# hamaadshah/gan_deeplearning4j

Hardware: NVIDIA H100
Metric: images/sec (full G+D step) (higher is better)
Workload: dtype bf16

## Files before the change

gan_deeplearning4j_b200/csrc/kernels_ew.cu:

```cuda
#include <stdlib.h>
#include <algorithm>
#include "kernels.h"
#include "common.cuh"

namespace b2g {

uint64_t g_launch_count = 0;
const char* g_ew_last_kernel = "";

template <typename T>
__global__ void nchw_f32_to_nhwc_kernel(const float* __restrict__ src, T* __restrict__ dst, int N, int C, int HW) { pdl_enter();
  size_t total = (size_t)N * C * HW;
  for (size_t i = blockIdx.x * (size_t)blockDim.x + threadIdx.x; i < total; i += (size_t)gridDim.x * blockDim.x) {
    int c = i % C; size_t t = i / C; int p = t % HW; size_t n = t / HW;
    stf(dst, i, src[(n * C + c) * HW + p]);
  }
}
template <typename T>
__global__ void nhwc_to_nchw_f32_kernel(const T* __restrict__ src, float* __restrict__ dst, int N, int C, int HW) { pdl_enter();
  size_t total = (size_t)N * C * HW;
  for (size_t i = blockIdx.x * (size_t)blockDim.x + threadIdx.x; i < total; i += (size_t)gridDim.x * blockDim.x) {
    int p = i % HW; size_t t = i / HW; int c = t % C; size_t n = t / C;
    dst[i] = ldf(src, (n * HW + p) * C + c);
  }
}
template <typename T>
__global__ void permute_kernel(const T* __restrict__ src, T* __restrict__ dst, int N, int C, int HW, int to_nhwc) { pdl_enter();
  size_t total = (size_t)N * C * HW;
  for (size_t i = blockIdx.x * (size_t)blockDim.x + threadIdx.x; i < total; i += (size_t)gridDim.x * blockDim.x) {
    if (to_nhwc) { int c = i % C; size_t t = i / C; int p = t % HW; size_t n = t / HW; dst[i] = src[(n * C + c) * HW + p]; }
    else         { int p = i % HW; size_t t = i / HW; int c = t % C; size_t n = t / C; dst[i] = src[(n * HW + p) * C + c]; }
  }
}
#define DISPATCH_ACT(act, ACTC, ...)                                                            \
  switch (act) {                                                                                \
    case ACT_IDENTITY: { constexpr int ACTC = ACT_IDENTITY; __VA_ARGS__; } break;               \
    case ACT_RELU: { constexpr int ACTC = ACT_RELU; __VA_ARGS__; } break;                       \
    case ACT_LRELU: { constexpr int ACTC = ACT_LRELU; __VA_ARGS__; } break;                     \
    default: { constexpr int ACTC = -1; __VA_ARGS__; } break;                                   \
  }
int device_sm_count() {
  static int sms[64] = {}; int d = 0; cudaGetDevice(&d); if (d < 0 || d >= 64) d = 0;
  if (!sms[d]) { int v = 0; cudaDeviceGetAttribute(&v, cudaDevAttrMultiProcessorCount, d); sms[d] = v > 0 ? v : 1; }
  return sms[d];
}
static inline int vec4_blocks(size_t n_vec) { const size_t cap = (size_t)device_sm_count() * 4; size_t b = (n_vec + 1023) / 1024; if (b > cap) b = cap; if (b < 1) b = 1; return (int)b; }
static inline int ew_blocks(size_t n, int per = 256) { const size_t cap = (size_t)device_sm_count() * 16; size_t b = (n + per - 1) / per; if (b > cap) b = cap; if (b < 1) b = 1; return (int)b; }

void k_nchw_f32_to_nhwc(int prec, const float* src, void* dst, int N, int C, int HW, cudaStream_t s) {
  size_t n = (size_t)N * C * HW; if (!n) return;
  DISPATCH_PREC(prec, T, (launch_pdl(nchw_f32_to_nhwc_kernel<T>, dim3(ew_blocks(n)), dim3(256), (size_t)(0), s, src, (T*)dst, N, C, HW))); LAUNCHED();
}
void k_nhwc_to_nchw_f32(int prec, const void* src, float* dst, int N, int C, int HW, cudaStream_t s) {
  size_t n = (size_t)N * C * HW; if (!n) return;
  DISPATCH_PREC(prec, T, (launch_pdl(nhwc_to_nchw_f32_kernel<T>, dim3(ew_blocks(n)), dim3(256), (size_t)(0), s, (const T*)src, dst, N, C, HW))); LAUNCHED();
}
void k_permute(int prec, const void* src, void* dst, int N, int C, int HW, int to_nhwc, cudaStream_t s) {
  size_t n = (size_t)N * C * HW; if (!n) return;
  DISPATCH_PREC(prec, T, (launch_pdl(permute_kernel<T>, dim3(ew_blocks(n)), dim3(256), (size_t)(0), s, (const T*)src, (T*)dst, N, C, HW, to_nhwc))); LAUNCHED();
}
__global__ void cast_f32_to_bf16_kernel(const float* __restrict__ src, __nv_bfloat16* __restrict__ dst, size_t n) { pdl_enter();
  for (size_t i = blockIdx.x * (size_t)blockDim.x + threadIdx.x; i < n; i += (size_t)gridDim.x * blockDim.x) dst[i] = __float2bfloat16_rn(src[i]);
}
void k_cast_f32_to_bf16(const float* src, __nv_bfloat16* dst, size_t n, cudaStream_t s) {
  if (!n) return; launch_pdl(cast_f32_to_bf16_kernel, dim3(ew_blocks(n)), dim3(256), (size_t)(0), s, src, dst, n); LAUNCHED();
}
static const int SLICE_ELEMS = 1 << 20;
static inline int pick_slices(int rows, int C) {
  int cap = SLICE_ELEMS / (C > 0 ? C : 1); if (cap < 1) cap = 1; if (cap > 2048) cap = 2048;
  int S = rows / 8; if (S < 1) S = 1; if (S > cap) S = cap; return S;
}
size_t k_bn_scratch_floats(int C, int groups) { return (size_t)2 * groups * (SLICE_ELEMS + 2 * (size_t)C) + 64; }
size_t k_colsum_scratch_floats(int C) { return (size_t)(SLICE_ELEMS + C) + 64; }

__device__ __forceinline__ void unpack8(const uint4& u, float (&v)[8]) {
  const __nv_bfloat162* h = reinterpret_cast<const __nv_bfloat162*>(&u);
#pragma unroll
  for (int j = 0; j < 4; ++j) { float2 f = __bfloat1622float2(h[j]); v[2 * j] = f.x; v[2 * j + 1] = f.y; }
}
__device__ __forceinline__ uint4 pack8(const float (&v)[8]) {
  uint4 u; __nv_bfloat162* h = reinterpret_cast<__nv_bfloat162*>(&u);
#pragma unroll
  for (int j = 0; j < 4; ++j) h[j] = __floats2bfloat162_rn(v[2 * j], v[2 * j + 1]);
  return u;
}

template <typename T>
__global__ void bn_stats_partial_kernel(const T* __restrict__ x, int rows, int C, int S, float* __restrict__ psum, float* __restrict__ psq, float* __restrict__ pivot) { pdl_enter();
  int g = blockIdx.y;
  int idx = blockIdx.x * blockDim.x + threadIdx.x;
  if (idx >= S * C) return;
  int c = idx % C, sl = idx / C;
  const T* xg = x + (size_t)g * rows * C;
  const float k = ldf(xg, c);
  if (sl == 0) pivot[g * C + c] = k;
  float a = 0.f, b = 0.f;
  for (int r = sl; r < rows; r += S) { float v = ldf(xg, (size_t)r * C + c) - k; a += v; b = fmaf(v, v, b); }
  psum[((size_t)g * S + sl) * C + c] = a; psq[((size_t)g * S + sl) * C + c] = b;
}
static inline int vec_ty(int C) { int c8 = C / 8; int ty = 256 / c8; return ty < 1 ? 1 : ty; }
static inline bool vec_ok(int prec, int C) { return prec == PREC_BF16 && C % 8 == 0 && C / 8 <= 256 && 256 % (C / 8) == 0; }
static inline int vec_blocks(int rows, int C) { int ty = vec_ty(C); int b = rows / (ty * 4); int cap = SLICE_ELEMS / C; if (cap > 256) cap = 256; if (b > cap) b = cap; if (b < 1) b = 1; return b; }
template <int NV>
__device__ __forceinline__ void block_fold_write(float (&acc)[NV][8], int C, int C8, int c8, int ty, int TY, float* const (&dst)[NV], size_t row_off) {
  __shared__ float sred[NV][2048];
#pragma unroll
  for (int v = 0; v < NV; ++v)
#pragma unroll
    for (int j = 0; j < 8; ++j) sred[v][ty * C + c8 * 8 + j] = acc[v][j];
  __syncthreads();
  for (int c = threadIdx.x; c < C; c += blockDim.x) {
#pragma unroll
    for (int v = 0; v < NV; ++v) { float a = 0.f; for (int k = 0; k < TY; ++k) a += sred[v][k * C + c]; dst[v][row_off + c] = a; }
  }
}
__global__ void __launch_bounds__(1024) bn_stats_final_kernel(const float* __restrict__ psum, const float* __restrict__ psq, const float* __restrict__ pivot, int rows, int C, int S, int groups, float eps,
                                      float* __restrict__ mean, float* __restrict__ invstd,
                                      const float* __restrict__ run_mean, const float* __restrict__ run_var, float* g_mean, float* g_var, float decay) { pdl_enter();
  __shared__ double sa[32][33], sb[32][33];
  const int tx = threadIdx.x & 31, ty = threadIdx.x >> 5, c = blockIdx.x * 32 + tx;
  double acc_gm = 0.0, acc_gv = 0.0;
  for (int g = 0; g < groups; ++g) {
    double a = 0.0, b = 0.0;
    if (c < C) for (int sl0 = ty; sl0 < S; sl0 += 32 * 8) {
      float va[8], vb[8];
#pragma unroll
      for (int q = 0; q < 8; ++q) { const int sl = sl0 + 32 * q; va[q] = sl < S ? psum[((size_t)g * S + sl) * C + c] : 0.f; vb[q] = sl < S ? psq[((size_t)g * S + sl) * C + c] : 0.f; }
#pragma unroll
      for (int q = 0; q < 8; ++q) { a += va[q]; b += vb[q]; }
    }
    sa[ty][tx] = a; sb[ty][tx] = b;
    __syncthreads();
    if (ty == 0 && c < C) {
      for (int k = 1; k < 32; ++k) { a += sa[k][tx]; b += sb[k][tx]; }
      const double d = a / rows, mu = (double)pivot[g * C + c] + d; double var = b / rows - d * d; if (var < 0) var = 0;
      mean[g * C + c] = (float)mu; invstd[g * C + c] = (float)(1.0 / sqrt(var + (double)eps));
      if (g_mean) { acc_gm += (1.0 - decay) * ((double)run_mean[c] - mu); acc_gv += (1.0 - decay) * ((double)run_var[c] - var); }
    }
    __syncthreads();
  }
  if (g_mean && ty == 0 && c < C) { g_mean[c] = (float)(acc_gm / groups); g_var[c] = (float)(acc_gv / groups); }
}
void k_bn_stats(int prec, const void* x, int rows, int C, int groups, float* scratch, float* mean, float* invstd, float eps,
                const float* run_mean, const float* run_var, float* g_mean, float* g_var, float decay, cudaStream_t s) {
  const int S = pick_slices(rows, C);
  float* psum = scratch; float* psq = scratch + (size_t)groups * S * C; float* pivot = psq + (size_t)groups * S * C;
  dim3 grid((S * C + 255) / 256, groups);
  DISPATCH_PREC(prec, T, (launch_pdl(bn_stats_partial_kernel<T>, dim3(grid), dim3(256), (size_t)(0), s, (const T*)x, rows, C, S, psum, psq, pivot)));
  LAUNCHED();
  launch_pdl(bn_stats_final_kernel, dim3((C + 31) / 32), dim3(1024), (size_t)(0), s, psum, psq, (const float*)pivot, rows, C, S, groups, eps, mean, invstd, run_mean, run_var, g_mean, g_var, decay); LAUNCHED();
}
__global__ void bn_prep_infer_kernel(const float* __restrict__ rm, const float* __restrict__ rv, int C, int groups, float eps, float* mean, float* invstd) { pdl_enter();
  int i = blockIdx.x * blockDim.x + threadIdx.x; if (i >= C * groups) return;
  int c = i % C; mean[i] = rm[c]; invstd[i] = 1.0f / sqrtf(rv[c] + eps);
}
__global__ void bn_fold_kernel(const float* __restrict__ rm, const float* __restrict__ rv, const float* __restrict__ gamma, const float* __restrict__ beta, const float* __restrict__ cb, int C, float eps, float* scale, float* shift) { pdl_enter();
  int c = blockIdx.x * blockDim.x + threadIdx.x; if (c >= C) return;
  const float sc = gamma[c] / sqrtf(rv[c] + eps); scale[c] = sc; shift[c] = beta[c] - rm[c] * sc + (cb ? cb[c] * sc : 0.f);
}
void k_bn_fold(const float* rm, const float* rv, const float* gamma, const float* beta, const float* cb, int C, float eps, float* scale, float* shift, cudaStream_t s) {
  launch_pdl(bn_fold_kernel, dim3((C + 255) / 256), dim3(256), (size_t)0, s, rm, rv, gamma, beta, cb, C, eps, scale, shift); LAUNCHED();
}
void k_bn_prep_infer(const float* run_mean, const float* run_var, int C, int groups, float eps, float* mean, float* invstd, cudaStream_t s) {
  launch_pdl(bn_prep_infer_kernel, dim3((C * groups + 255) / 256), dim3(256), (size_t)(0), s, run_mean, run_var, C, groups, eps, mean, invstd); LAUNCHED();
}

template <typename T>
__global__ void bn_apply_kernel(const T* __restrict__ x, T* __restrict__ y, int rows, int C, int groups, const float* __restrict__ mean,
                                const float* __restrict__ invstd, const float* __restrict__ gamma, const float* __restrict__ beta, int act, float alpha) { pdl_enter();
  size_t per_group = (size_t)rows * C, total = per_group * groups;
  for (size_t i = blockIdx.x * (size_t)blockDim.x + threadIdx.x; i < total; i += (size_t)gridDim.x * blockDim.x) {
    int c = i % C; int g = i / per_group;
    float v = (ldf(x, i) - mean[g * C + c]) * invstd[g * C + c];
    stf(y, i, act_fwd(act, fmaf(gamma[c], v, beta[c]), alpha));
  }
}
template <int ACTC>
__global__ void __launch_bounds__(256, 3) bn_apply_bf16x8_kernel(const uint4* __restrict__ x, uint4* __restrict__ y, int rows, int C, int groups, const float* __restrict__ mean,
                                       const float* __restrict__ invstd, const float* __restrict__ gamma, const float* __restrict__ beta, int act, float alpha) { pdl_enter();
  const int C8 = C / 8; const size_t per_group = (size_t)rows * C8;
  const size_t t0 = blockIdx.x * (size_t)blockDim.x + threadIdx.x, stride = (size_t)gridDim.x * blockDim.x;
  const int c0 = (int)(t0 % C8) * 8;
  for (int g = 0; g < groups; ++g) {
    float mu[8], is[8], ga[8], be[8];
#pragma unroll
    for (int j = 0; j < 8; ++j) { mu[j] = mean[g * C + c0 + j]; is[j] = invstd[g * C + c0 + j]; ga[j] = gamma[c0 + j]; be[j] = beta[c0 + j]; }
    const uint4* xg = x + g * per_group; uint4* yg = y + g * per_group;
    for (size_t i = t0; i < per_group; i += 4 * stride) {
      uint4 xa[4];
#pragma unroll
      for (int q = 0; q < 4; ++q) if (i + q * stride < per_group) xa[q] = xg[i + q * stride];
#pragma unroll
      for (int q = 0; q < 4; ++q) if (i + q * stride < per_group) {
        float v[8]; unpack8(xa[q], v);
#pragma unroll
        for (int j = 0; j < 8; ++j) v[j] = act_fwd(ACTC < 0 ? act : ACTC, fmaf(ga[j], (v[j] - mu[j]) * is[j], be[j]), alpha);
        yg[i + q * stride] = pack8(v);
      }
    }
  }
}
void k_bn_apply(int prec, const void* x, void* y, int rows, int C, int groups, const float* mean, const float* invstd,
                const float* gamma, const float* beta, int act, float alpha, cudaStream_t s) {
  size_t n = (size_t)rows * C * groups; if (!n) return;
  if (vec_ok(prec, C)) {
    DISPATCH_ACT(act, ACTC, launch_pdl(bn_apply_bf16x8_kernel<ACTC>, dim3(vec4_blocks((size_t)rows * C / 8)), dim3(256), (size_t)(0), s, (const uint4*)x, (uint4*)y, rows, C, groups, mean, invstd, gamma, beta, act, alpha));
  } else {
    DISPATCH_PREC(prec, T, (launch_pdl(bn_apply_kernel<T>, dim3(ew_blocks(n)), dim3(256), (size_t)(0), s, (const T*)x, (T*)y, rows, C, groups, mean, invstd, gamma, beta, act, alpha)));
  }
  LAUNCHED();
}

template <typename T>
__global__ void bn_bwd_partial_kernel(const T* __restrict__ x, const T* __restrict__ eo, int rows, int C, int S, const float* __restrict__ mean,
                                      const float* __restrict__ invstd, const float* __restrict__ gamma, const float* __restrict__ beta, int act, float alpha,
                                      float* __restrict__ p1, float* __restrict__ p2) { pdl_enter();
  int g = blockIdx.y;
  int idx = blockIdx.x * blockDim.x + threadIdx.x;
  if (idx >= S * C) return;
  int c = idx % C, sl = idx / C;
  const T* xg = x + (size_t)g * rows * C; const T* eg = eo + (size_t)g * rows * C;
  float mu = mean[g * C + c], is = invstd[g * C + c], ga = gamma[c], be = beta[c];
  float a = 0.f, b = 0.f;
  for (int r = sl; r < rows; r += S) {
    float xh = (ldf(xg, (size_t)r * C + c) - mu) * is;
    float dy = ldf(eg, (size_t)r * C + c) * act_grad_from_pre(act, fmaf(ga, xh, be), alpha);
    a += dy; b = fmaf(dy, xh, b);
  }
  p1[((size_t)g * S + sl) * C + c] = a; p2[((size_t)g * S + sl) * C + c] = b;
}
__global__ void __launch_bounds__(1024) bn_bwd_final_kernel(const float* __restrict__ p1, const float* __restrict__ p2, int rows, int C, int S, int groups,
                                    float* __restrict__ c1, float* __restrict__ c2, float* g_gamma, float* g_beta, int want) { pdl_enter();
  __shared__ double sa[32][33], sb[32][33];
  const int tx = threadIdx.x & 31, ty = threadIdx.x >> 5, c = blockIdx.x * 32 + tx;
  double tg = 0.0, tb = 0.0;
  for (int g = 0; g < groups; ++g) {
    double a = 0.0, b = 0.0;
    if (c < C) for (int sl0 = ty; sl0 < S; sl0 += 32 * 8) {
      float va[8], vb[8];
#pragma unroll
      for (int q = 0; q < 8; ++q) { const int sl = sl0 + 32 * q; va[q] = sl < S ? p1[((size_t)g * S + sl) * C + c] : 0.f; vb[q] = sl < S ? p2[((size_t)g * S + sl) * C + c] : 0.f; }
#pragma unroll
      for (int q = 0; q < 8; ++q) { a += va[q]; b += vb[q]; }
    }
    sa[ty][tx] = a; sb[ty][tx] = b;
    __syncthreads();
    if (ty == 0 && c < C) {
      for (int k = 1; k < 32; ++k) { a += sa[k][tx]; b += sb[k][tx]; }
      c1[g * C + c] = (float)(a / rows); c2[g * C + c] = (float)(b / rows); tb += a; tg += b;
    }
    __syncthreads();
  }
  if (want && ty == 0 && c < C) { g_beta[c] += (float)tb; g_gamma[c] += (float)tg; }
}
template <typename T>
__global__ void bn_bwd_apply_kernel(const T* __restrict__ x, const T* __restrict__ eo, T* __restrict__ ei, int rows, int C, int groups,
                                    const float* __restrict__ mean, const float* __restrict__ invstd, const float* __restrict__ gamma,
                                    const float* __restrict__ beta, int act, float alpha, const float* __restrict__ c1, const float* __restrict__ c2) { pdl_enter();
  size_t per_group = (size_t)rows * C, total = per_group * groups;
  for (size_t i = blockIdx.x * (size_t)blockDim.x + threadIdx.x; i < total; i += (size_t)gridDim.x * blockDim.x) {
    int c = i % C; int g = i / per_group; int k = g * C + c;
    float xh = (ldf(x, i) - mean[k]) * invstd[k];
    float dy = ldf(eo, i) * act_grad_from_pre(act, fmaf(gamma[c], xh, beta[c]), alpha);
    stf(ei, i, gamma[c] * invstd[k] * (dy - c1[k] - xh * c2[k]));
  }
}
void k_bn_bwd(int prec, const void* x, const void* eps_out, void* eps_in, int rows, int C, int groups,
              const float* mean, const float* invstd, const float* gamma, const float* beta, int act, float alpha,
              float* scratch, float* g_gamma, float* g_beta, int want, cudaStream_t s) {
  const int S = pick_slices(rows, C);
  float* p1 = scratch; float* p2 = p1 + (size_t)groups * S * C; float* c1 = p2 + (size_t)groups * S * C; float* c2 = c1 + (size_t)groups * C;
  dim3 grid((S * C + 255) / 256, groups);
  DISPATCH_PREC(prec, T, (launch_pdl(bn_bwd_partial_kernel<T>, dim3(grid), dim3(256), (size_t)(0), s, (const T*)x, (const T*)eps_out, rows, C, S, mean, invstd, gamma, beta, act, alpha, p1, p2)));
  LAUNCHED();
  launch_pdl(bn_bwd_final_kernel, dim3((C + 31) / 32), dim3(1024), (size_t)(0), s, p1, p2, rows, C, S, groups, c1, c2, g_gamma, g_beta, want); LAUNCHED();
  if (eps_in) {
    size_t n = (size_t)rows * C * groups;
    DISPATCH_PREC(prec, T, (launch_pdl(bn_bwd_apply_kernel<T>, dim3(ew_blocks(n)), dim3(256), (size_t)(0), s, (const T*)x, (const T*)eps_out, (T*)eps_in, rows, C, groups, mean, invstd, gamma, beta, act, alpha, c1, c2)));
    LAUNCHED();
  }
}


bool k_bn_vec_ok(int prec, int C) { return vec_ok(prec, C); }
size_t k_bn_acc_elems(int C, int groups) { return (size_t)groups * 4 * C; }

template <int NV, typename A>
__device__ __forceinline__ void block_fold_acc(A (&acc)[NV][8], int C, int c8, int ty, int TY, unsigned long long* accbase ) {
  __shared__ double sred[NV][2048];
#pragma unroll
  for (int v = 0; v < NV; ++v)
#pragma unroll
    for (int j = 0; j < 8; ++j) sred[v][ty * C + c8 * 8 + j] = acc[v][j];
  __syncthreads();
  for (int c = threadIdx.x; c < C; c += blockDim.x) {
#pragma unroll
    for (int v = 0; v < NV; ++v) { double a = 0.0; for (int k = 0; k < TY; ++k) a += sred[v][k * C + c]; sacc_add(accbase + (size_t)v * 2 * C, (size_t)C, (size_t)c, a); }
  }
}
__global__ void __launch_bounds__(256) bn_stats_acc_kernel(const uint4* __restrict__ x, int rows, int C, int S, unsigned long long* __restrict__ accp) { pdl_enter();
  const int g = blockIdx.y, C8 = C / 8, TY = 256 / C8, c8 = threadIdx.x % C8, ty = threadIdx.x / C8, sl = blockIdx.x;
  const int chunk = (rows + S - 1) / S, r0 = sl * chunk, r1 = min(rows, r0 + chunk);
  const uint4* xg = x + (size_t)g * rows * C8;
  double acc[2][8];
#pragma unroll
  for (int j = 0; j < 8; ++j) { acc[0][j] = 0.0; acc[1][j] = 0.0; }
#pragma unroll 4
  for (int r = r0 + ty; r < r1; r += TY) { float v[8]; unpack8(xg[(size_t)r * C8 + c8], v);
#pragma unroll
    for (int j = 0; j < 8; ++j) { acc[0][j] += v[j]; acc[1][j] = fma((double)v[j], (double)v[j], acc[1][j]); } }
  block_fold_acc<2>(acc, C, c8, ty, TY, accp + (size_t)g * 4 * C);
}
void k_bn_stats_acc(const void* x, int rows, int C, int groups, unsigned long long* acc, cudaStream_t s) {
  const int S = vec_blocks(rows, C);
  launch_pdl(bn_stats_acc_kernel, dim3(S, groups), dim3(256), (size_t)0, s, (const uint4*)x, rows, C, S, acc); LAUNCHED();
}

__device__ __forceinline__ float bn_pre_act(int act, float x, float sc, float be, float mu) {
  return (act == ACT_RELU || act == ACT_LRELU) ? fmaf(x, sc, fmaf(-mu, sc, be)) : fmaf(x - mu, sc, be);
}
template <int ACTC>
__global__ void __launch_bounds__(256, 3) bn_apply_acc_kernel(const uint4* __restrict__ x, uint4* __restrict__ y, int rows, int C, int groups, const unsigned long long* __restrict__ accp,
                                                             const float* __restrict__ gamma, const float* __restrict__ beta, int act, float alpha, float eps, float* __restrict__ coef,
                                                             const float* __restrict__ run_mean, const float* __restrict__ run_var, float* g_mean, float* g_var, float decay, int replicas) { pdl_enter();
  extern __shared__ float s_cf[];
  const double cnt = (double)rows * replicas, inv_cnt = 1.0 / cnt;
  const bool writer = blockIdx.x == 0;
  const int C8 = C / 8; const size_t per_group = (size_t)rows * C8;
  const size_t t0 = blockIdx.x * (size_t)blockDim.x + threadIdx.x, stride = (size_t)gridDim.x * blockDim.x;
  uint4 xa[4];
#pragma unroll
  for (int q = 0; q < 4; ++q) if (t0 + q * stride < per_group) xa[q] = x[t0 + q * stride];
  for (int c = threadIdx.x; c < C; c += blockDim.x) {
    double agm = 0.0, agv = 0.0;
    for (int g = 0; g < groups; ++g) {
      const unsigned long long* a = accp + (size_t)g * 4 * C;
      const double mu = sacc_read(a, (size_t)C, (size_t)c) * inv_cnt; double var = sacc_read(a + 2 * (size_t)C, (size_t)C, (size_t)c) * inv_cnt - mu * mu; if (var < 0) var = 0;
      const float is = (float)(1.0 / sqrt(var + (double)eps)), sc = gamma[c] * is, sh = fmaf(-(float)mu, sc, beta[c]);
      s_cf[(g * 2 + 0) * C + c] = sc; s_cf[(g * 2 + 1) * C + c] = sh;
      if (writer) {
        coef[(size_t)(g * 4 + 0) * C + c] = sc; coef[(size_t)(g * 4 + 1) * C + c] = beta[c]; coef[(size_t)(g * 4 + 2) * C + c] = (float)mu; coef[(size_t)(g * 4 + 3) * C + c] = is;
        if (g_mean) { agm += (1.0 - decay) * ((double)run_mean[c] - mu); agv += (1.0 - decay) * ((double)run_var[c] - var); }
      }
    }
    if (writer && g_mean) { g_mean[c] = (float)(agm / groups); g_var[c] = (float)(agv / groups); }
  }
  __syncthreads();
  const int c0 = (int)(t0 % C8) * 8;
  bool preloaded = true;
  for (int g = 0; g < groups; ++g) {
    float sc[8], sh[8];
#pragma unroll
    for (int j = 0; j < 8; ++j) { sc[j] = s_cf[(g * 2 + 0) * C + c0 + j]; sh[j] = s_cf[(g * 2 + 1) * C + c0 + j]; }
    const uint4* xg = x + g * per_group; uint4* yg = y + g * per_group;
    for (size_t i = t0; i < per_group; i += 4 * stride) {
      if (!preloaded) {
#pragma unroll
        for (int q = 0; q < 4; ++q) if (i + q * stride < per_group) xa[q] = xg[i + q * stride];
      }
      preloaded = false;
#pragma unroll
      for (int q = 0; q < 4; ++q) if (i + q * stride < per_group) {
        float v[8]; unpack8(xa[q], v);
#pragma unroll
        for (int j = 0; j < 8; ++j) v[j] = act_fwd(ACTC < 0 ? act : ACTC, fmaf(v[j], sc[j], sh[j]), alpha);
        yg[i + q * stride] = pack8(v);
      }
    }
  }
}
void k_bn_apply_acc(const void* x, void* y, int rows, int C, int groups, const unsigned long long* acc, const float* gamma, const float* beta, int act, float alpha, float eps,
                    float* coef, const float* run_mean, const float* run_var, float* g_mean, float* g_var, float decay, cudaStream_t s, int replicas) {
  const size_t smem = sizeof(float) * 2 * groups * C;
  DISPATCH_ACT(act, ACTC, launch_pdl(bn_apply_acc_kernel<ACTC>, dim3(vec4_blocks((size_t)rows * C / 8)), dim3(256), smem, s, (const uint4*)x, (uint4*)y, rows, C, groups, acc, gamma, beta, act, alpha, eps,
                                     coef, run_mean, run_var, g_mean, g_var, decay, replicas));
  LAUNCHED();
}

template <int ACTC>
__global__ void __launch_bounds__(256, 3) bn_bwd_stats_acc_kernel(const uint4* __restrict__ x, const uint4* __restrict__ eo, int rows, int C, int S, const float* __restrict__ coef,
                                                                 int act, float alpha, unsigned long long* __restrict__ accp) { pdl_enter();
  const int g = blockIdx.y, C8 = C / 8, TY = 256 / C8, c8 = threadIdx.x % C8, ty = threadIdx.x / C8, sl = blockIdx.x;
  const int chunk = (rows + S - 1) / S, r0 = sl * chunk, r1 = min(rows, r0 + chunk);
  const uint4* xg = x + (size_t)g * rows * C8; const uint4* eg = eo + (size_t)g * rows * C8;
  float sc[8], be[8], mu[8], is[8], acc[2][8];
#pragma unroll
  for (int j = 0; j < 8; ++j) { const int c = c8 * 8 + j; sc[j] = coef[(size_t)(g * 4 + 0) * C + c]; be[j] = coef[(size_t)(g * 4 + 1) * C + c]; mu[j] = coef[(size_t)(g * 4 + 2) * C + c]; is[j] = coef[(size_t)(g * 4 + 3) * C + c]; acc[0][j] = 0.f; acc[1][j] = 0.f; }
#pragma unroll 4
  for (int r = r0 + ty; r < r1; r += TY) {
    float xv[8], ev[8]; unpack8(xg[(size_t)r * C8 + c8], xv); unpack8(eg[(size_t)r * C8 + c8], ev);
#pragma unroll
    for (int j = 0; j < 8; ++j) { const float xh = (xv[j] - mu[j]) * is[j]; const float dy = ev[j] * act_grad_from_pre(ACTC < 0 ? act : ACTC, bn_pre_act(ACTC < 0 ? act : ACTC, xv[j], sc[j], be[j], mu[j]), alpha); acc[0][j] += dy; acc[1][j] = fmaf(dy, xh, acc[1][j]); }
  }
  block_fold_acc<2>(acc, C, c8, ty, TY, accp + (size_t)g * 4 * C);
}
void k_bn_bwd_stats_acc(const void* x, const void* eps_out, int rows, int C, int groups, const float* coef, int act, float alpha, unsigned long long* acc, cudaStream_t s) {
  const int S = vec_blocks(rows, C);
  DISPATCH_ACT(act, ACTC, launch_pdl(bn_bwd_stats_acc_kernel<ACTC>, dim3(S, groups), dim3(256), (size_t)0, s, (const uint4*)x, (const uint4*)eps_out, rows, C, S, coef, act, alpha, acc));
  LAUNCHED();
}

template <int ACTC, bool PREMUL>
__global__ void __launch_bounds__(256, 2) bn_bwd_apply_acc_kernel(const uint4* __restrict__ x, const uint4* __restrict__ eo, uint4* __restrict__ ei, int rows, int C, int groups,
                                                                 const float* __restrict__ coef, int act, float alpha, const unsigned long long* __restrict__ accp,
                                                                 float* g_gamma, float* g_beta, int want, int replicas) { pdl_enter();
  extern __shared__ float s_k[];
  const double cnt = (double)rows * replicas, inv_cnt = 1.0 / cnt;
  const bool writer = blockIdx.x == 0 && want;
  const int C8 = C / 8; const size_t per_group = (size_t)rows * C8;
  const size_t t0 = blockIdx.x * (size_t)blockDim.x + threadIdx.x, stride = (size_t)gridDim.x * blockDim.x;
  uint4 xa[4], ea[4];
  if (ei) {
#pragma unroll
    for (int q = 0; q < 4; ++q) if (t0 + q * stride < per_group) { xa[q] = x[t0 + q * stride]; ea[q] = eo[t0 + q * stride]; }
  }
  for (int c = threadIdx.x; c < C; c += blockDim.x) {
    double tb = 0.0, tg = 0.0;
    for (int g = 0; g < groups; ++g) {
      const unsigned long long* a = accp + (size_t)g * 4 * C;
      const double s1 = sacc_read(a, (size_t)C, (size_t)c); double s2 = sacc_read(a + 2 * (size_t)C, (size_t)C, (size_t)c);
      if (PREMUL) s2 = (double)coef[(size_t)(g * 4 + 3) * C + c] * (s2 - (double)coef[(size_t)(g * 4 + 2) * C + c] * s1);
      s_k[(g * 2 + 0) * C + c] = (float)(s1 * inv_cnt); s_k[(g * 2 + 1) * C + c] = (float)(s2 * inv_cnt); tb += s1; tg += s2;
    }
    if (writer) { g_beta[c] += (float)(tb / replicas); g_gamma[c] += (float)(tg / replicas); }
  }
  __syncthreads();
  if (!ei) return;
  const int c0 = (int)(t0 % C8) * 8;
  bool preloaded = true;
  for (int g = 0; g < groups; ++g) {
    float sc[8], be[8], mu[8], is[8], k1[8], k2[8];
#pragma unroll
    for (int j = 0; j < 8; ++j) { const int c = c0 + j; sc[j] = coef[(size_t)(g * 4 + 0) * C + c]; be[j] = coef[(size_t)(g * 4 + 1) * C + c]; mu[j] = coef[(size_t)(g * 4 + 2) * C + c]; is[j] = coef[(size_t)(g * 4 + 3) * C + c];
      k1[j] = s_k[(g * 2 + 0) * C + c]; k2[j] = s_k[(g * 2 + 1) * C + c]; }
    const uint4* xg = x + g * per_group; const uint4* eg = eo + g * per_group; uint4* ig = ei + g * per_group;
    for (size_t i = t0; i < per_group; i += 4 * stride) {
      if (!preloaded) {
#pragma unroll
        for (int q = 0; q < 4; ++q) if (i + q * stride < per_group) { xa[q] = xg[i + q * stride]; ea[q] = eg[i + q * stride]; }
      }
      preloaded = false;
#pragma unroll
      for (int q = 0; q < 4; ++q) if (i + q * stride < per_group) {
        float xv[8], ev[8], o[8]; unpack8(xa[q], xv); unpack8(ea[q], ev);
#pragma unroll
        for (int j = 0; j < 8; ++j) { const float xh = (xv[j] - mu[j]) * is[j];
          const float dy = PREMUL ? ev[j] : ev[j] * act_grad_from_pre(ACTC < 0 ? act : ACTC, bn_pre_act(ACTC < 0 ? act : ACTC, xv[j], sc[j], be[j], mu[j]), alpha); o[j] = sc[j] * (dy - k1[j] - xh * k2[j]); }
        ig[i + q * stride] = pack8(o);
      }
    }
  }
}
void k_bn_bwd_apply_acc(const void* x, const void* eps_out, void* eps_in, int rows, int C, int groups, const float* coef, int act, float alpha, int premul,
                        const unsigned long long* acc, float* g_gamma, float* g_beta, int want, cudaStream_t s, int replicas) {
  const size_t smem = sizeof(float) * 2 * groups * C;
  const dim3 grid(eps_in ? vec4_blocks((size_t)rows * C / 8) : 1);
  if (premul) { launch_pdl(bn_bwd_apply_acc_kernel<ACT_IDENTITY, true>, grid, dim3(256), smem, s, (const uint4*)x, (const uint4*)eps_out, (uint4*)eps_in, rows, C, groups, coef, act, alpha, acc, g_gamma, g_beta, want, replicas); }
  else { DISPATCH_ACT(act, ACTC, launch_pdl(bn_bwd_apply_acc_kernel<ACTC, false>, grid, dim3(256), smem, s, (const uint4*)x, (const uint4*)eps_out, (uint4*)eps_in, rows, C, groups, coef, act, alpha, acc, g_gamma, g_beta, want, replicas)); }
  LAUNCHED();
}


__device__ __forceinline__ void st_release_sys(unsigned* p, unsigned v) { asm volatile("st.release.sys.global.u32 [%0], %1;" ::"l"(p), "r"(v) : "memory"); }
__device__ __forceinline__ unsigned ld_acquire_sys(const unsigned* p) { unsigned v; asm volatile("ld.acquire.sys.global.u32 %0, [%1];" : "=r"(v) : "l"(p) : "memory"); return v; }
__device__ __forceinline__ void p2p_wait_all(const unsigned* flags, int world, unsigned e) {
  for (int r = 0; r < world; ++r) {
    unsigned it = 0;
    while ((int)(ld_acquire_sys(flags + r) - e) < 0) { if (++it > (1u << 27)) __trap(); __nanosleep(32); }
  }
}
__global__ void __launch_bounds__(512) p2p_allreduce_kernel(const P2pArgs a) {
  __shared__ unsigned s_e;
  if (threadIdx.x == 0) s_e = *reinterpret_cast<volatile unsigned*>(a.state) + 1;
  __syncthreads();
  const unsigned e = s_e; const int W = a.world;
  unsigned* mine = a.flags[a.rank];
  if (blockIdx.x == 0 && threadIdx.x < W) st_release_sys(a.flags[threadIdx.x] + a.rank, e);
  if (threadIdx.x == 0) p2p_wait_all(mine, W, e);
  __syncthreads();
  const size_t nv = a.n / 4, chunk = (nv + W - 1) / W, v0 = min(nv, (size_t)a.rank * chunk), v1 = min(nv, v0 + chunk);
  for (size_t i = v0 + blockIdx.x * (size_t)blockDim.x + threadIdx.x; i < v1; i += (size_t)gridDim.x * blockDim.x) {
    float4 acc = __ldcg(reinterpret_cast<const float4*>(a.grads[0]) + i);
    for (int r = 1; r < W; ++r) { const float4 v = __ldcg(reinterpret_cast<const float4*>(a.grads[r]) + i); acc.x += v.x; acc.y += v.y; acc.z += v.z; acc.w += v.w; }
    for (int r = 0; r < W; ++r) __stcg(reinterpret_cast<float4*>(a.grads[r]) + i, acc);
  }
  if (a.rank == W - 1 && blockIdx.x == 0 && threadIdx.x < (a.n & 3)) {
    const size_t i = nv * 4 + threadIdx.x; float acc = __ldcg(a.grads[0] + i);
    for (int r = 1; r < W; ++r) acc += __ldcg(a.grads[r] + i);
    for (int r = 0; r < W; ++r) __stcg(a.grads[r] + i, acc);
  }
  __threadfence_system();
  __syncthreads();
  if (threadIdx.x == 0) {
    const unsigned t = atomicAdd(a.state + 1, 1u);
    if (t == gridDim.x - 1) {
      a.state[1] = 0;
      for (int r = 0; r < W; ++r) st_release_sys(a.flags[r] + 8 + a.rank, e);
      p2p_wait_all(mine + 8, W, e);
      *reinterpret_cast<volatile unsigned*>(a.state) = e;
      __threadfence();
    }
  }
}
void k_p2p_allreduce(const P2pArgs& a, cudaStream_t s) {
  const size_t slice = (a.n / 4 + a.world - 1) / a.world;
  int blocks = (int)((slice + 2047) / 2048); if (blocks > 120) blocks = 120; if (blocks < 1) blocks = 1;
  p2p_allreduce_kernel<<<blocks, 512, 0, s>>>(a); LAUNCHED();
}

template <typename T>
__global__ void act_fwd_kernel(const T* __restrict__ x, T* __restrict__ y, size_t n, int act, float alpha) { pdl_enter();
  for (size_t i = blockIdx.x * (size_t)blockDim.x + threadIdx.x; i < n; i += (size_t)gridDim.x * blockDim.x) stf(y, i, act_fwd(act, ldf(x, i), alpha));
}
template <typename T>
__global__ void act_bwd_out_kernel(const T* __restrict__ a, const T* __restrict__ eo, T* __restrict__ ei, size_t n, int act, float alpha) { pdl_enter();
  for (size_t i = blockIdx.x * (size_t)blockDim.x + threadIdx.x; i < n; i += (size_t)gridDim.x * blockDim.x)
    stf(ei, i, ldf(eo, i) * act_grad_from_out(act, ldf(a, i), alpha));
}
void k_act_fwd(int prec, const void* x, void* y, size_t n, int act, float alpha, cudaStream_t s) {
  if (!n) return; DISPATCH_PREC(prec, T, (launch_pdl(act_fwd_kernel<T>, dim3(ew_blocks(n)), dim3(256), (size_t)(0), s, (const T*)x, (T*)y, n, act, alpha))); LAUNCHED();
  g_ew_last_kernel = "act_fwd_kernel";
}
template <int ACTC>
__global__ void __launch_bounds__(256, 4) act_bwd_out_bf16x8_kernel(const uint4* __restrict__ a, const uint4* __restrict__ eo, uint4* __restrict__ ei, size_t n8, int act, float alpha) { pdl_enter();
  const size_t stride = (size_t)gridDim.x * blockDim.x;
  for (size_t i = blockIdx.x * (size_t)blockDim.x + threadIdx.x; i < n8; i += 4 * stride) {
    uint4 aa[4], ea[4];
#pragma unroll
    for (int q = 0; q < 4; ++q) if (i + q * stride < n8) { aa[q] = a[i + q * stride]; ea[q] = eo[i + q * stride]; }
#pragma unroll
    for (int q = 0; q < 4; ++q) if (i + q * stride < n8) {
      float av[8], ev[8], o[8]; unpack8(aa[q], av); unpack8(ea[q], ev);
#pragma unroll
      for (int j = 0; j < 8; ++j) o[j] = ev[j] * act_grad_from_out(ACTC < 0 ? act : ACTC, av[j], alpha);
      ei[i + q * stride] = pack8(o);
    }
  }
}
void k_act_bwd_from_output(int prec, const void* a, const void* eo, void* ei, size_t n, int act, float alpha, cudaStream_t s) {
  if (!n) return;
  if (prec == PREC_BF16 && n % 8 == 0 && ((reinterpret_cast<uintptr_t>(a) | reinterpret_cast<uintptr_t>(eo) | reinterpret_cast<uintptr_t>(ei)) & 15) == 0) {
    DISPATCH_ACT(act, ACTC, launch_pdl(act_bwd_out_bf16x8_kernel<ACTC>, dim3(vec4_blocks(n / 8)), dim3(256), (size_t)0, s, (const uint4*)a, (const uint4*)eo, (uint4*)ei, n / 8, act, alpha)); LAUNCHED();
    g_ew_last_kernel = "act_bwd_out_bf16x8_kernel"; return;
  }
  DISPATCH_PREC(prec, T, (launch_pdl(act_bwd_out_kernel<T>, dim3(ew_blocks(n)), dim3(256), (size_t)(0), s, (const T*)a, (const T*)eo, (T*)ei, n, act, alpha))); LAUNCHED();
  g_ew_last_kernel = "act_bwd_out_kernel";
}
void k_sigmoid_out(int prec, const void* z, void* p, size_t n, cudaStream_t s) { k_act_fwd(prec, z, p, n, ACT_SIGMOID, 0.f, s); }

template <typename T>
__global__ void maxpool_fwd_kernel(const T* __restrict__ x, T* __restrict__ y, uint8_t* __restrict__ arg, int N, int H, int W, int C, int OH, int OW, int KH, int KW, int SH, int SW) { pdl_enter();
  size_t total = (size_t)N * OH * OW * C;
  for (size_t i = blockIdx.x * (size_t)blockDim.x + threadIdx.x; i < total; i += (size_t)gridDim.x * blockDim.x) {
    int c = i % C; size_t t = i / C; int ox = t % OW; t /= OW; int oy = t % OH; size_t n = t / OH;
    float best = -INFINITY; int bi = 0;
    for (int r = 0; r < KH; ++r) for (int q = 0; q < KW; ++q) {
      float v = ldf(x, ((n * H + oy * SH + r) * W + ox * SW + q) * C + c);
      if (v > best) { best = v; bi = r * KW + q; }
    }
    stf(y, i, best); arg[i] = (uint8_t)bi;
  }
}
template <typename T>
__global__ void maxpool_bwd_kernel(const T* __restrict__ eo, const uint8_t* __restrict__ arg, T* __restrict__ ei, int N, int H, int W, int C, int OH, int OW, int KH, int KW, int SH, int SW) { pdl_enter();
  size_t total = (size_t)N * H * W * C;
  for (size_t i = blockIdx.x * (size_t)blockDim.x + threadIdx.x; i < total; i += (size_t)gridDim.x * blockDim.x) {
    int c = i % C; size_t t = i / C; int ix = t % W; t /= W; int iy = t % H; size_t n = t / H;
    float acc = 0.f;
    for (int r = 0; r < KH; ++r) { int ty = iy - r; if (ty < 0 || ty % SH) continue; int oy = ty / SH; if (oy >= OH) continue;
      for (int q = 0; q < KW; ++q) { int tx = ix - q; if (tx < 0 || tx % SW) continue; int ox = tx / SW; if (ox >= OW) continue;
        size_t o = ((n * OH + oy) * OW + ox) * C + c;
        if (arg[o] == r * KW + q) acc += ldf(eo, o);
      } }
    stf(ei, i, acc);
  }
}
void k_maxpool_fwd(int prec, const void* x, void* y, uint8_t* arg, int N, int H, int W, int C, int OH, int OW, int KH, int KW, int SH, int SW, cudaStream_t s) {
  size_t n = (size_t)N * OH * OW * C; if (!n) return;
  DISPATCH_PREC(prec, T, (launch_pdl(maxpool_fwd_kernel<T>, dim3(ew_blocks(n)), dim3(256), (size_t)(0), s, (const T*)x, (T*)y, arg, N, H, W, C, OH, OW, KH, KW, SH, SW))); LAUNCHED();
  g_ew_last_kernel = "maxpool_fwd_kernel";
}
void k_maxpool_bwd(int prec, const void* eo, const uint8_t* arg, void* ei, int N, int H, int W, int C, int OH, int OW, int KH, int KW, int SH, int SW, cudaStream_t s) {
  size_t n = (size_t)N * H * W * C; if (!n) return;
  DISPATCH_PREC(prec, T, (launch_pdl(maxpool_bwd_kernel<T>, dim3(ew_blocks(n)), dim3(256), (size_t)(0), s, (const T*)eo, arg, (T*)ei, N, H, W, C, OH, OW, KH, KW, SH, SW))); LAUNCHED();
  g_ew_last_kernel = "maxpool_bwd_kernel";
}
template <typename T>
__global__ void upsample_fwd_kernel(const T* __restrict__ x, T* __restrict__ y, int N, int H, int W, int C, int f) { pdl_enter();
  size_t total = (size_t)N * H * f * W * f * C;
  for (size_t i = blockIdx.x * (size_t)blockDim.x + threadIdx.x; i < total; i += (size_t)gridDim.x * blockDim.x) {
    int c = i % C; size_t t = i / C; int ox = t % (W * f); t /= (W * f); int oy = t % (H * f); size_t n = t / (H * f);
    y[i] = x[((n * H + oy / f) * W + ox / f) * C + c];
  }
}
template <typename T>
__global__ void upsample_bwd_kernel(const T* __restrict__ eo, T* __restrict__ ei, int N, int H, int W, int C, int f) { pdl_enter();
  size_t total = (size_t)N * H * W * C;
  for (size_t i = blockIdx.x * (size_t)blockDim.x + threadIdx.x; i < total; i += (size_t)gridDim.x * blockDim.x) {
    int c = i % C; size_t t = i / C; int ix = t % W; t /= W; int iy = t % H; size_t n = t / H;
    float acc = 0.f;
    for (int a = 0; a < f; ++a) for (int b = 0; b < f; ++b) acc += ldf(eo, ((n * H * f + iy * f + a) * (size_t)(W * f) + ix * f + b) * C + c);
    stf(ei, i, acc);
  }
}
void k_upsample_fwd(int prec, const void* x, void* y, int N, int H, int W, int C, int f, cudaStream_t s) {
  size_t n = (size_t)N * H * f * W * f * C; if (!n) return;
  DISPATCH_PREC(prec, T, (launch_pdl(upsample_fwd_kernel<T>, dim3(ew_blocks(n)), dim3(256), (size_t)(0), s, (const T*)x, (T*)y, N, H, W, C, f))); LAUNCHED();
  g_ew_last_kernel = "upsample_fwd_kernel";
}
void k_upsample_bwd(int prec, const void* eo, void* ei, int N, int H, int W, int C, int f, cudaStream_t s) {
  size_t n = (size_t)N * H * W * C; if (!n) return;
  DISPATCH_PREC(prec, T, (launch_pdl(upsample_bwd_kernel<T>, dim3(ew_blocks(n)), dim3(256), (size_t)(0), s, (const T*)eo, (T*)ei, N, H, W, C, f))); LAUNCHED();
  g_ew_last_kernel = "upsample_bwd_kernel";
}

template <typename T>
__global__ void xent_kernel(const T* __restrict__ z, const float* __restrict__ y, T* __restrict__ dz, float* __restrict__ loss_sums, int rows, float clip) { pdl_enter();
  int g = blockIdx.x;
  __shared__ double red[32];
  double acc = 0.0;
  for (int r = threadIdx.x; r < rows; r += blockDim.x) {
    size_t i = (size_t)g * rows + r;
    float zi = ldf(z, i), yi = y[i], loss, grad;
    float sg = 1.0f / (1.0f + expf(-zi));
    if (clip > 0.f) {
      float p = fminf(fmaxf(sg, clip), 1.0f - clip);
      loss = -(yi * logf(p) + (1.0f - yi) * logf(1.0f - p));
      grad = (p - yi) / (p * (1.0f - p)) * sg * (1.0f - sg);
    } else {
      loss = fmaxf(zi, 0.f) + log1pf(expf(-fabsf(zi))) - yi * zi;
      grad = sg - yi;
    }
    acc += loss; stf(dz, i, grad);
  }
  for (int o = 16; o; o >>= 1) acc += __shfl_xor_sync(0xffffffffu, acc, o);
  if (threadIdx.x % 32 == 0) red[threadIdx.x / 32] = acc;
  __syncthreads();
  if (threadIdx.x == 0) { double t = 0; for (int w = 0; w < (blockDim.x + 31) / 32; ++w) t += red[w]; loss_sums[g] = (float)t; }
}
void k_xent(int prec, const void* z, const float* y, void* dz, float* loss_sums, int rows, int groups, float clip, cudaStream_t s) {
  DISPATCH_PREC(prec, T, (launch_pdl(xent_kernel<T>, dim3(groups), dim3(1024), (size_t)(0), s, (const T*)z, y, (T*)dz, loss_sums, rows, clip))); LAUNCHED();
  g_ew_last_kernel = "xent_kernel";
}

template <typename T>
__global__ void softmax_xent_kernel(const T* __restrict__ z, const float* __restrict__ y, T* __restrict__ dz, T* __restrict__ p_out, float* __restrict__ loss_sum, int rows, int K) { pdl_enter();
  __shared__ double red[32];
  double acc = 0.0;
  for (int r = threadIdx.x; r < rows; r += blockDim.x) {
    float m = -INFINITY; for (int k = 0; k < K; ++k) m = fmaxf(m, ldf(z, (size_t)r * K + k));
    float den = 0.f; for (int k = 0; k < K; ++k) den += expf(ldf(z, (size_t)r * K + k) - m);
    for (int k = 0; k < K; ++k) {
      const float p = expf(ldf(z, (size_t)r * K + k) - m) / den;
      if (p_out) stf(p_out, (size_t)r * K + k, p);
      if (dz) { const float yk = y[(size_t)r * K + k]; stf(dz, (size_t)r * K + k, p - yk); acc -= (double)yk * log((double)fminf(fmaxf(p, 1e-10f), 1.0f - 1e-10f)); }
    }
  }
  for (int o = 16; o; o >>= 1) acc += __shfl_xor_sync(0xffffffffu, acc, o);
  if (threadIdx.x % 32 == 0) red[threadIdx.x / 32] = acc;
  __syncthreads();
  if (threadIdx.x == 0 && loss_sum) { double t = 0; for (int w = 0; w < (blockDim.x + 31) / 32; ++w) t += red[w]; loss_sum[0] = (float)t; }
}
void k_softmax_xent(int prec, const void* z, const float* y, void* dz, void* p_out, float* loss_sums, int rows, int K, cudaStream_t s) {
  DISPATCH_PREC(prec, T, (launch_pdl(softmax_xent_kernel<T>, dim3(1), dim3(1024), (size_t)0, s, (const T*)z, y, (T*)dz, (T*)p_out, loss_sums, rows, K))); LAUNCHED();
  g_ew_last_kernel = "softmax_xent_kernel";
}

constexpr int LOSS_THREADS = 256, LOSS_ELEMS_PER_BLOCK = 1024, LOSS_MAX_GRID = 1024;
int k_loss_blocks(size_t n_per_group, int groups) {
  const size_t b = (n_per_group + LOSS_ELEMS_PER_BLOCK - 1) / LOSS_ELEMS_PER_BLOCK;
  return (int)std::min<size_t>(std::max<size_t>(b, 1), std::max(1, LOSS_MAX_GRID / groups));
}
template <typename T>
__global__ void __launch_bounds__(LOSS_THREADS) loss_kernel(const T* __restrict__ z, const float* __restrict__ y, T* __restrict__ dz, float* __restrict__ loss_sums,
                                                           size_t n_per_group, int n_out, int bpg, int loss, int act, float alpha, double* partial, unsigned* ticket) {
  pdl_enter();
  __shared__ double red[LOSS_THREADS / 32];
  __shared__ int last;
  const int g = blockIdx.x / bpg, b = blockIdx.x % bpg;
  const float nf = (float)n_out;
  double acc = 0.0;
  for (size_t j = (size_t)b * LOSS_THREADS + threadIdx.x; j < n_per_group; j += (size_t)bpg * LOSS_THREADS) {
    const size_t i = (size_t)g * n_per_group + j;
    const float a = act_fwd(act, ldf(z, i), alpha), yi = y[i];
    const double e = (double)a - (double)yi, m = 1.0 - (double)yi * (double)a;
    double l; float ga;
    switch (loss) {
      case LOSS_MSE: l = e * e; ga = 2.0f * (a - yi) / nf; break;
      case LOSS_L2: l = e * e; ga = 2.0f * (a - yi); break;
      case LOSS_L1: l = fabs(e); ga = (float)((a > yi) - (a < yi)); break;
      case LOSS_MAE: l = fabs(e); ga = (float)((a > yi) - (a < yi)) / nf; break;
      case LOSS_HINGE: l = fmax(m, 0.0); ga = m > 0.0 ? -yi : 0.f; break;
      case LOSS_SQUARED_HINGE: l = m > 0.0 ? m * m : 0.0; ga = m > 0.0 ? -2.0f * yi * (float)m : 0.f; break;
      default: l = (double)yi * (double)a; ga = yi / nf; break;
    }
    acc += l;
    stf(dz, i, ga * act_grad_from_out(act, a, alpha));
  }
  const double tot = block_sum(acc, red);
  if (threadIdx.x == 0) {
    partial[blockIdx.x] = tot;
    __threadfence();
    last = atomicAdd(ticket, 1u) == gridDim.x - 1;
  }
  __syncthreads();
  if (!last) return;
  __threadfence();
  const bool per_out = loss == LOSS_MSE || loss == LOSS_MAE || loss == LOSS_WASSERSTEIN;
  const int warp = threadIdx.x >> 5, lane = threadIdx.x & 31;
  for (int gg = warp; gg < (int)(gridDim.x / bpg); gg += LOSS_THREADS / 32) {
    double s = 0.0;
    for (int k = lane; k < bpg; k += 32) s += __ldcg(partial + (size_t)gg * bpg + k);
#pragma unroll
    for (int o = 16; o > 0; o >>= 1) s += __shfl_xor_sync(0xffffffffu, s, o);
    if (lane == 0) loss_sums[gg] = (float)(per_out ? s / n_out : s);
  }
  if (threadIdx.x == 0) { *ticket = 0u; __threadfence(); }
}
void k_loss(int prec, int loss, int act, float alpha, const void* z, const float* y, void* dz, float* loss_sums, int rows_per_group, int n_out, int groups,
            double* partial, unsigned* ticket, cudaStream_t s) {
  const size_t n = (size_t)rows_per_group * n_out; const int bpg = k_loss_blocks(n, groups);
  DISPATCH_PREC(prec, T, (launch_pdl(loss_kernel<T>, dim3(groups * bpg), dim3(LOSS_THREADS), (size_t)0, s, (const T*)z, y, (T*)dz, loss_sums, n, n_out, bpg,
                                     loss, act, alpha, partial, ticket))); LAUNCHED();
  g_ew_last_kernel = "loss_kernel";
}

template <typename T>
__global__ void colsum_partial_kernel(const T* __restrict__ x, int rows, int C, int S, float* __restrict__ p) { pdl_enter();
  int idx = blockIdx.x * blockDim.x + threadIdx.x; if (idx >= S * C) return;
  int c = idx % C, sl = idx / C; float a = 0.f;
  for (int r = sl; r < rows; r += S) a += ldf(x, (size_t)r * C + c);
  p[(size_t)sl * C + c] = a;
}
__global__ void __launch_bounds__(256) colsum_partial_bf16x8_kernel(const uint4* __restrict__ x, int rows, int C, int S, float* __restrict__ p) { pdl_enter();
  const int C8 = C / 8, TY = 256 / C8, c8 = threadIdx.x % C8, ty = threadIdx.x / C8, sl = blockIdx.x;
  const int chunk = (rows + S - 1) / S, r0 = sl * chunk, r1 = min(rows, r0 + chunk);
  float acc[1][8];
#pragma unroll
  for (int j = 0; j < 8; ++j) acc[0][j] = 0.f;
  for (int r = r0 + ty; r < r1; r += TY) { float v[8]; unpack8(x[(size_t)r * C8 + c8], v);
#pragma unroll
    for (int j = 0; j < 8; ++j) acc[0][j] += v[j]; }
  float* const dst[1] = {p};
  block_fold_write<1>(acc, C, C8, c8, ty, TY, dst, (size_t)sl * C);
}
__global__ void __launch_bounds__(512) colsum_final_kernel(const float* __restrict__ p, int C, int S, float* out, int accumulate) { pdl_enter();
  __shared__ double sa[16][33];
  const int tx = threadIdx.x & 31, ty = threadIdx.x >> 5, c = blockIdx.x * 32 + tx;
  double a = 0.0;
  if (c < C) for (int sl0 = ty; sl0 < S; sl0 += 16 * 8) {
    float va[8];
#pragma unroll
    for (int q = 0; q < 8; ++q) { const int sl = sl0 + 16 * q; va[q] = sl < S ? p[(size_t)sl * C + c] : 0.f; }
#pragma unroll
    for (int q = 0; q < 8; ++q) a += va[q];
  }
  sa[ty][tx] = a;
  __syncthreads();
  if (ty == 0 && c < C) { for (int k = 1; k < 16; ++k) a += sa[k][tx]; out[c] = (accumulate ? out[c] : 0.f) + (float)a; }
}
template <int C>
// ... 251 lines not shown
```

Baseline: 92300.

## Flatten BN apply kernels over groups with wave-sized grids and shared coefficients

The forward and backward BN apply kernels now walk one flattened index space across all groups, finding each element's group on the fly, instead of looping over groups per thread. Grids are sized from the total element count and capped at a few waves of SMs. The backward kernel also stages the per-group coefficients (scale, beta, mean, inv-std) in shared memory and reads them with vector loads, reloading only when the group changes. This aims to balance work across groups and cut repeated global coefficient loads, at the cost of a per-element group lookup and more shared memory (which may need the opt-in attribute for large C).

```diff
diff --git a/gan_deeplearning4j_b200/csrc/kernels_ew.cu b/gan_deeplearning4j_b200/csrc/kernels_ew.cu
--- a/gan_deeplearning4j_b200/csrc/kernels_ew.cu
+++ b/gan_deeplearning4j_b200/csrc/kernels_ew.cu
@@ -319,18 +319,28 @@
 __device__ __forceinline__ float bn_pre_act(int act, float x, float sc, float be, float mu) {
   return (act == ACT_RELU || act == ACT_LRELU) ? fmaf(x, sc, fmaf(-mu, sc, be)) : fmaf(x - mu, sc, be);
 }
+static inline int bn_wave_blocks(size_t n_vec, int per_sm) {
+  const size_t cap = (size_t)device_sm_count() * per_sm; size_t b = (n_vec + 1023) / 1024; if (b > cap) b = cap; if (b < 1) b = 1; return (int)b;
+}
+__device__ __forceinline__ int bn_group_of(size_t k, size_t per_group) { int g = 0; for (size_t r = per_group; k >= r; r += per_group) ++g; return g; }
+__device__ __forceinline__ void ld8_shared(const float* p, float (&v)[8]) {
+  const float4 a = reinterpret_cast<const float4*>(p)[0], b = reinterpret_cast<const float4*>(p)[1];
+  v[0] = a.x; v[1] = a.y; v[2] = a.z; v[3] = a.w; v[4] = b.x; v[5] = b.y; v[6] = b.z; v[7] = b.w;
+}
+template <typename K>
+static inline void allow_dyn_smem(K* kernel, size_t smem) { if (smem > 48 * 1024) cudaFuncSetAttribute(kernel, cudaFuncAttributeMaxDynamicSharedMemorySize, (int)smem); }
 template <int ACTC>
 __global__ void __launch_bounds__(256, 3) bn_apply_acc_kernel(const uint4* __restrict__ x, uint4* __restrict__ y, int rows, int C, int groups, const unsigned long long* __restrict__ accp,
                                                              const float* __restrict__ gamma, const float* __restrict__ beta, int act, float alpha, float eps, float* __restrict__ coef,
                                                              const float* __restrict__ run_mean, const float* __restrict__ run_var, float* g_mean, float* g_var, float decay, int replicas) { pdl_enter();
-  extern __shared__ float s_cf[];
+  extern __shared__ __align__(16) float s_cf[];
   const double cnt = (double)rows * replicas, inv_cnt = 1.0 / cnt;
   const bool writer = blockIdx.x == 0;
-  const int C8 = C / 8; const size_t per_group = (size_t)rows * C8;
+  const int C8 = C / 8; const size_t per_group = (size_t)rows * C8, total = per_group * groups;
   const size_t t0 = blockIdx.x * (size_t)blockDim.x + threadIdx.x, stride = (size_t)gridDim.x * blockDim.x;
   uint4 xa[4];
 #pragma unroll
-  for (int q = 0; q < 4; ++q) if (t0 + q * stride < per_group) xa[q] = x[t0 + q * stride];
+  for (int q = 0; q < 4; ++q) if (t0 + q * stride < total) xa[q] = x[t0 + q * stride];
   for (int c = threadIdx.x; c < C; c += blockDim.x) {
     double agm = 0.0, agv = 0.0;
     for (int g = 0; g < groups; ++g) {
@@ -347,32 +357,28 @@
   }
   __syncthreads();
   const int c0 = (int)(t0 % C8) * 8;
-  bool preloaded = true;
-  for (int g = 0; g < groups; ++g) {
-    float sc[8], sh[8];
-#pragma unroll
-    for (int j = 0; j < 8; ++j) { sc[j] = s_cf[(g * 2 + 0) * C + c0 + j]; sh[j] = s_cf[(g * 2 + 1) * C + c0 + j]; }
-    const uint4* xg = x + g * per_group; uint4* yg = y + g * per_group;
-    for (size_t i = t0; i < per_group; i += 4 * stride) {
-      if (!preloaded) {
-#pragma unroll
-        for (int q = 0; q < 4; ++q) if (i + q * stride < per_group) xa[q] = xg[i + q * stride];
-      }
-      preloaded = false;
-#pragma unroll
-      for (int q = 0; q < 4; ++q) if (i + q * stride < per_group) {
-        float v[8]; unpack8(xa[q], v);
-#pragma unroll
-        for (int j = 0; j < 8; ++j) v[j] = act_fwd(ACTC < 0 ? act : ACTC, fmaf(v[j], sc[j], sh[j]), alpha);
-        yg[i + q * stride] = pack8(v);
-      }
+  for (size_t i = t0; i < total; i += 4 * stride) {
+    if (i != t0) {
+#pragma unroll
+      for (int q = 0; q < 4; ++q) if (i + q * stride < total) xa[q] = x[i + q * stride];
+    }
+#pragma unroll
+    for (int q = 0; q < 4; ++q) if (i + q * stride < total) {
+      const size_t k = i + q * stride; const int g = bn_group_of(k, per_group);
+      const float4* sc4 = reinterpret_cast<const float4*>(s_cf + (size_t)(g * 2 + 0) * C + c0); const float4* sh4 = reinterpret_cast<const float4*>(s_cf + (size_t)(g * 2 + 1) * C + c0);
+      const float4 a0 = sc4[0], a1 = sc4[1], b0 = sh4[0], b1 = sh4[1];
+      const float sc[8] = {a0.x, a0.y, a0.z, a0.w, a1.x, a1.y, a1.z, a1.w}, sh[8] = {b0.x, b0.y, b0.z, b0.w, b1.x, b1.y, b1.z, b1.w};
+      float v[8]; unpack8(xa[q], v);
+#pragma unroll
+      for (int j = 0; j < 8; ++j) v[j] = act_fwd(ACTC < 0 ? act : ACTC, fmaf(v[j], sc[j], sh[j]), alpha);
+      y[k] = pack8(v);
     }
   }
 }
 void k_bn_apply_acc(const void* x, void* y, int rows, int C, int groups, const unsigned long long* acc, const float* gamma, const float* beta, int act, float alpha, float eps,
                     float* coef, const float* run_mean, const float* run_var, float* g_mean, float* g_var, float decay, cudaStream_t s, int replicas) {
   const size_t smem = sizeof(float) * 2 * groups * C;
-  DISPATCH_ACT(act, ACTC, launch_pdl(bn_apply_acc_kernel<ACTC>, dim3(vec4_blocks((size_t)rows * C / 8)), dim3(256), smem, s, (const uint4*)x, (uint4*)y, rows, C, groups, acc, gamma, beta, act, alpha, eps,
+  DISPATCH_ACT(act, ACTC, launch_pdl(bn_apply_acc_kernel<ACTC>, dim3(bn_wave_blocks((size_t)rows * C / 8 * groups, 3)), dim3(256), smem, s, (const uint4*)x, (uint4*)y, rows, C, groups, acc, gamma, beta, act, alpha, eps,
                                      coef, run_mean, run_var, g_mean, g_var, decay, replicas));
   LAUNCHED();
 }
@@ -404,15 +410,15 @@
 __global__ void __launch_bounds__(256, 2) bn_bwd_apply_acc_kernel(const uint4* __restrict__ x, const uint4* __restrict__ eo, uint4* __restrict__ ei, int rows, int C, int groups,
                                                                  const float* __restrict__ coef, int act, float alpha, const unsigned long long* __restrict__ accp,
                                                                  float* g_gamma, float* g_beta, int want, int replicas) { pdl_enter();
-  extern __shared__ float s_k[];
+  extern __shared__ __align__(16) float s_k[];
   const double cnt = (double)rows * replicas, inv_cnt = 1.0 / cnt;
   const bool writer = blockIdx.x == 0 && want;
-  const int C8 = C / 8; const size_t per_group = (size_t)rows * C8;
+  const int C8 = C / 8; const size_t per_group = (size_t)rows * C8, total = per_group * groups;
   const size_t t0 = blockIdx.x * (size_t)blockDim.x + threadIdx.x, stride = (size_t)gridDim.x * blockDim.x;
   uint4 xa[4], ea[4];
   if (ei) {
 #pragma unroll
-    for (int q = 0; q < 4; ++q) if (t0 + q * stride < per_group) { xa[q] = x[t0 + q * stride]; ea[q] = eo[t0 + q * stride]; }
+    for (int q = 0; q < 4; ++q) if (t0 + q * stride < total) { xa[q] = x[t0 + q * stride]; ea[q] = eo[t0 + q * stride]; }
   }
   for (int c = threadIdx.x; c < C; c += blockDim.x) {
     double tb = 0.0, tg = 0.0;
@@ -420,43 +426,46 @@
       const unsigned long long* a = accp + (size_t)g * 4 * C;
       const double s1 = sacc_read(a, (size_t)C, (size_t)c); double s2 = sacc_read(a + 2 * (size_t)C, (size_t)C, (size_t)c);
       if (PREMUL) s2 = (double)coef[(size_t)(g * 4 + 3) * C + c] * (s2 - (double)coef[(size_t)(g * 4 + 2) * C + c] * s1);
-      s_k[(g * 2 + 0) * C + c] = (float)(s1 * inv_cnt); s_k[(g * 2 + 1) * C + c] = (float)(s2 * inv_cnt); tb += s1; tg += s2;
+      s_k[(g * 6 + 0) * C + c] = (float)(s1 * inv_cnt); s_k[(g * 6 + 1) * C + c] = (float)(s2 * inv_cnt); tb += s1; tg += s2;
+      if (ei) {
+#pragma unroll
+        for (int r = 0; r < 4; ++r) s_k[(g * 6 + 2 + r) * C + c] = coef[(size_t)(g * 4 + r) * C + c];
+      }
     }
     if (writer) { g_beta[c] += (float)(tb / replicas); g_gamma[c] += (float)(tg / replicas); }
   }
   __syncthreads();
   if (!ei) return;
   const int c0 = (int)(t0 % C8) * 8;
-  bool preloaded = true;
-  for (int g = 0; g < groups; ++g) {
-    float sc[8], be[8], mu[8], is[8], k1[8], k2[8];
-#pragma unroll
-    for (int j = 0; j < 8; ++j) { const int c = c0 + j; sc[j] = coef[(size_t)(g * 4 + 0) * C + c]; be[j] = coef[(size_t)(g * 4 + 1) * C + c]; mu[j] = coef[(size_t)(g * 4 + 2) * C + c]; is[j] = coef[(size_t)(g * 4 + 3) * C + c];
-      k1[j] = s_k[(g * 2 + 0) * C + c]; k2[j] = s_k[(g * 2 + 1) * C + c]; }
-    const uint4* xg = x + g * per_group; const uint4* eg = eo + g * per_group; uint4* ig = ei + g * per_group;
-    for (size_t i = t0; i < per_group; i += 4 * stride) {
-      if (!preloaded) {
-#pragma unroll
-        for (int q = 0; q < 4; ++q) if (i + q * stride < per_group) { xa[q] = xg[i + q * stride]; ea[q] = eg[i + q * stride]; }
+  float k1[8], k2[8], sc[8], be[8], mu[8], is[8];
+  int gc = -1;
+  for (size_t i = t0; i < total; i += 4 * stride) {
+    if (i != t0) {
+#pragma unroll
+      for (int q = 0; q < 4; ++q) if (i + q * stride < total) { xa[q] = x[i + q * stride]; ea[q] = eo[i + q * stride]; }
+    }
+#pragma unroll
+    for (int q = 0; q < 4; ++q) if (i + q * stride < total) {
+      const size_t k = i + q * stride; const int g = bn_group_of(k, per_group);
+      if (g != gc) {
+        gc = g;
+        ld8_shared(s_k + (size_t)(g * 6 + 0) * C + c0, k1); ld8_shared(s_k + (size_t)(g * 6 + 1) * C + c0, k2); ld8_shared(s_k + (size_t)(g * 6 + 2) * C + c0, sc);
+        ld8_shared(s_k + (size_t)(g * 6 + 3) * C + c0, be); ld8_shared(s_k + (size_t)(g * 6 + 4) * C + c0, mu); ld8_shared(s_k + (size_t)(g * 6 + 5) * C + c0, is);
       }
-      preloaded = false;
-#pragma unroll
-      for (int q = 0; q < 4; ++q) if (i + q * stride < per_group) {
-        float xv[8], ev[8], o[8]; unpack8(xa[q], xv); unpack8(ea[q], ev);
-#pragma unroll
-        for (int j = 0; j < 8; ++j) { const float xh = (xv[j] - mu[j]) * is[j];
-          const float dy = PREMUL ? ev[j] : ev[j] * act_grad_from_pre(ACTC < 0 ? act : ACTC, bn_pre_act(ACTC < 0 ? act : ACTC, xv[j], sc[j], be[j], mu[j]), alpha); o[j] = sc[j] * (dy - k1[j] - xh * k2[j]); }
-        ig[i + q * stride] = pack8(o);
-      }
+      float xv[8], ev[8], o[8]; unpack8(xa[q], xv); unpack8(ea[q], ev);
+#pragma unroll
+      for (int j = 0; j < 8; ++j) { const float xh = (xv[j] - mu[j]) * is[j];
+        const float dy = PREMUL ? ev[j] : ev[j] * act_grad_from_pre(ACTC < 0 ? act : ACTC, bn_pre_act(ACTC < 0 ? act : ACTC, xv[j], sc[j], be[j], mu[j]), alpha); o[j] = sc[j] * (dy - k1[j] - xh * k2[j]); }
+      ei[k] = pack8(o);
     }
   }
 }
 void k_bn_bwd_apply_acc(const void* x, const void* eps_out, void* eps_in, int rows, int C, int groups, const float* coef, int act, float alpha, int premul,
                         const unsigned long long* acc, float* g_gamma, float* g_beta, int want, cudaStream_t s, int replicas) {
-  const size_t smem = sizeof(float) * 2 * groups * C;
-  const dim3 grid(eps_in ? vec4_blocks((size_t)rows * C / 8) : 1);
-  if (premul) { launch_pdl(bn_bwd_apply_acc_kernel<ACT_IDENTITY, true>, grid, dim3(256), smem, s, (const uint4*)x, (const uint4*)eps_out, (uint4*)eps_in, rows, C, groups, coef, act, alpha, acc, g_gamma, g_beta, want, replicas); }
-  else { DISPATCH_ACT(act, ACTC, launch_pdl(bn_bwd_apply_acc_kernel<ACTC, false>, grid, dim3(256), smem, s, (const uint4*)x, (const uint4*)eps_out, (uint4*)eps_in, rows, C, groups, coef, act, alpha, acc, g_gamma, g_beta, want, replicas)); }
+  const size_t smem = sizeof(float) * 6 * groups * C;
+  const dim3 grid(eps_in ? bn_wave_blocks((size_t)rows * C / 8 * groups, 2) : 1);
+  if (premul) { allow_dyn_smem(bn_bwd_apply_acc_kernel<ACT_IDENTITY, true>, smem); launch_pdl(bn_bwd_apply_acc_kernel<ACT_IDENTITY, true>, grid, dim3(256), smem, s, (const uint4*)x, (const uint4*)eps_out, (uint4*)eps_in, rows, C, groups, coef, act, alpha, acc, g_gamma, g_beta, want, replicas); }
+  else { DISPATCH_ACT(act, ACTC, allow_dyn_smem(bn_bwd_apply_acc_kernel<ACTC, false>, smem); launch_pdl(bn_bwd_apply_acc_kernel<ACTC, false>, grid, dim3(256), smem, s, (const uint4*)x, (const uint4*)eps_out, (uint4*)eps_in, rows, C, groups, coef, act, alpha, acc, g_gamma, g_beta, want, replicas)); }
   LAUNCHED();
 }
 
```

Result: faster. 93280, median of 6 (+1.1%).
